# ejcanalesr/multicomponent-T2-toolbox

Hardware: AMD Instinct MI355X
Metric: voxels/sec (whole node) at nTE=32, nT2=60; max |MWF-ref| (higher is better)
Workload: dtype f64

## Files before the change

### include/met2_hip.h

```cpp
#ifndef MET2_HIP_H
#define MET2_HIP_H

#include <stdint.h>

#ifdef __cplusplus
extern "C" {
#endif

#define MET2_ABI_VERSION 6

enum met2_method {
    MET2_NNLS = 0,
    MET2_T2SPARC = 1,
    MET2_X2 = 2,
    MET2_LCURVE = 3,
    MET2_GCV = 4,
    MET2_BAYESREG = 5
};

enum met2_penalty { MET2_PEN_I = 0, MET2_PEN_L1 = 1, MET2_PEN_L2 = 2, MET2_PEN_INVT2 = 3 };

enum met2_status {
    MET2_ST_FITTED = 1,
    MET2_ST_ITMAX = 2,
// ... 112 lines not shown
int met2_fa_bruteforce_strided(met2_plan *plan, int64_t nvox, const double *data, int64_t voxel_stride, int64_t echo_stride,
                               const uint8_t *mask, double *fa_index, double *km, double *resid, void *stream);

int met2_fa_spline_select(int32_t device, int64_t nvox, int32_t n_lr, const double *alpha_lr, const double *resid,
                          int32_t n_hr, const double *alpha_hr, int32_t n_te, const double *data, const uint8_t *mask,
                          double *fa_index, double *xmin, void *stream);

int met2_fa_spline_select_strided(int32_t device, int64_t nvox, int32_t n_lr, const double *alpha_lr, const double *resid,
                                  int32_t n_hr, const double *alpha_hr, int32_t n_te, const double *data, int64_t voxel_stride,
                                  int64_t echo_stride, const uint8_t *mask, double *fa_index, double *xmin, void *stream);

int met2_smooth_separable(int32_t device, int32_t nx, int32_t ny, int32_t nz, int32_t n_te, int32_t radius, const double *weights,
                          const double *data, double *out, double *work, void *stream);

int met2_nesma(int32_t device, int32_t nx, int32_t ny, int32_t nz, int32_t n_te, const double *data,
               const uint8_t *mask, double *out, void *stream);

int64_t met2_tv_work_bytes(int32_t nx, int32_t ny, int32_t nz, int32_t n_te, int32_t echo_major);
int met2_tv_chambolle(int32_t device, int32_t nx, int32_t ny, int32_t nz, int32_t n_te, const double *data, int32_t echo_major,
                      const double *weight, double weight_factor, double eps, int32_t max_num_iter, int32_t poll_every, double *out,
                      double *sigma, int32_t *iters, void *work, int64_t work_bytes, void *stream);
int met2_tv_last_timing(double *iter_ms, int32_t *launches);

int met2_roi_reduce(met2_plan *src, met2_plan *dst, int64_t nvox, const double *data, int64_t voxel_stride, int64_t echo_stride,
                    const int32_t *roi_index, const double *fa_index, double *mean_signal, double *count, void *stream);

int met2_metrics(met2_plan *plan, int64_t nvox, const double *fsol, const uint8_t *mask, double *maps,
                 void *stream);

int met2_plan_last_kernel_ms(met2_plan *plan, double *ms);
int met2_plan_last_spill_count(met2_plan *plan, int64_t *count);
int met2_plan_last_second_pass_ms(met2_plan *plan, double *ms);

int met2_plan_launch_info(met2_plan *plan, int32_t method, int32_t *grid, int32_t *block, int32_t *lds_bytes);

int met2_plan_gcv_form(met2_plan *plan, int32_t *low_rank, double *residual);

#ifdef __cplusplus
}
#endif
#endif
```

### multicomponent-t2-toolbox_amd/_lib.py

```python
import ctypes as C
import os

from . import _build

_LIB = None

_dp = C.POINTER(C.c_double)


class Met2Error(RuntimeError):
    pass


class Options(C.Structure):
    _fields_ = [("struct_size", C.c_int32), ("device", C.c_int32), ("x2_factor", C.c_double), ("t2sparc_lambda", C.c_double),
                ("brent_xtol", C.c_double), ("brent_maxfun", C.c_int32), ("reserved0", C.c_int32), ("t2_myelin_cut", C.c_double),
                ("t2_ie_cut", C.c_double), ("x2_lo", C.c_double), ("x2_hi", C.c_double), ("gcv_lo", C.c_double), ("gcv_hi", C.c_double),
                ("bayes_lo", C.c_double), ("bayes_hi", C.c_double)]


class SynthParams(C.Structure):
    _fields_ = [("struct_size", C.c_int32), ("reserved0", C.c_int32), ("te", C.c_double), ("TR", C.c_double), ("T1", C.c_double)] + [
        (k, C.c_double) for k in ("mwf_lo", "mwf_hi", "t2m_lo", "t2m_hi", "t2ie_lo", "t2ie_hi", "fa_lo", "fa_hi", "snr_lo", "snr_hi", "sm_lo", "sm_hi",
                                  "sie_lo", "sie_hi", "km")]


SYMBOLS = ["met2_default_options", "met2_abi_version", "met2_device_count", "met2_last_error", "met2_plan_create",
           "met2_plan_destroy", "met2_plan_set_options", "met2_plan_get_options", "met2_plan_build_dictionary_epg", "met2_plan_set_dictionary", "met2_plan_get_dictionary",
           "met2_plan_set_penalty", "met2_plan_set_penalty_dense", "met2_plan_get_penalty", "met2_plan_set_lambda_grid",
           "met2_plan_set_t2_grid", "met2_fit", "met2_fit_strided", "met2_fit_enqueue_strided", "met2_plan_finish", "met2_fa_bruteforce", "met2_fa_bruteforce_strided", "met2_fa_spline_select",
           "met2_fa_spline_select_strided", "met2_roi_reduce", "met2_nesma", "met2_tv_work_bytes", "met2_tv_chambolle", "met2_tv_last_timing", "met2_smooth_separable", "met2_metrics", "met2_plan_last_kernel_ms", "met2_plan_last_second_pass_ms", "met2_plan_last_spill_count",
           "met2_plan_launch_info", "met2_plan_gcv_form", "met2_plan_get_shape", "met2_fit_host", "met2_plan_attach_fa_spline", "met2_host_trim",
           "met2_fit_bootstrap", "met2_bootstrap_replicates", "met2_synth_two_lobe", "met2_eval_voxel_metrics", "met2_eval_reduce"]


def lib():
    global _LIB
    if _LIB is None:
        path = _build.LIB
        if not os.path.exists(path):
            raise Met2Error("HIP extension %s is not built (run __graft_entry__.build()); there is no CPU fallback" % path)
        L = C.CDLL(path)
        L.met2_last_error.restype = C.c_char_p
        vp = C.c_void_p
        L.met2_plan_create.argtypes = [C.POINTER(vp), C.c_int32, C.c_int32, C.c_int32, C.POINTER(Options)]
        L.met2_plan_destroy.argtypes = [vp]
        L.met2_plan_set_options.argtypes = [vp, C.POINTER(Options)]
        L.met2_plan_get_options.argtypes = [vp, C.POINTER(Options)]
        L.met2_plan_build_dictionary_epg.argtypes = [vp, _dp, _dp, C.c_double, _dp, C.c_double, vp]
        L.met2_plan_set_dictionary.argtypes = [vp, _dp]
        L.met2_plan_get_dictionary.argtypes = [vp, _dp]
        L.met2_plan_set_penalty.argtypes = [vp, C.c_int32, _dp]
        L.met2_plan_set_penalty_dense.argtypes = [vp, _dp]
        L.met2_plan_get_penalty.argtypes = [vp, _dp]
        L.met2_plan_set_lambda_grid.argtypes = [vp, _dp, C.c_int32]
        L.met2_plan_set_t2_grid.argtypes = [vp, _dp]
        L.met2_fit.argtypes = [vp, C.c_int32, C.c_int64] + [vp] * 10
        L.met2_fit_strided.argtypes = [vp, C.c_int32, C.c_int64, vp, C.c_int64, C.c_int64] + [vp] * 9
        L.met2_fit_enqueue_strided.argtypes = [vp, C.c_int32, C.c_int64, vp, C.c_int64, C.c_int64] + [vp] * 9
        L.met2_plan_finish.argtypes = [vp, vp]
        L.met2_fa_bruteforce.argtypes = [vp, C.c_int64] + [vp] * 6
        L.met2_fa_bruteforce_strided.argtypes = [vp, C.c_int64, vp, C.c_int64, C.c_int64] + [vp] * 5
        L.met2_fa_spline_select_strided.argtypes = [C.c_int32, C.c_int64, C.c_int32, _dp, vp, C.c_int32, _dp, C.c_int32, vp, C.c_int64, C.c_int64,
                                                    vp, vp, vp, vp]
        L.met2_roi_reduce.argtypes = [vp, vp, C.c_int64, vp, C.c_int64, C.c_int64, vp, vp, vp, vp, vp]
        L.met2_fa_spline_select.argtypes = [C.c_int32, C.c_int64, C.c_int32, _dp, vp, C.c_int32, _dp, C.c_int32, vp, vp, vp, vp, vp]
        L.met2_nesma.argtypes = [C.c_int32] * 5 + [vp] * 4
        L.met2_tv_work_bytes.argtypes = [C.c_int32] * 5
        L.met2_tv_work_bytes.restype = C.c_int64
        L.met2_tv_chambolle.argtypes = [C.c_int32] * 5 + [vp, C.c_int32, _dp, C.c_double, C.c_double, C.c_int32, C.c_int32, vp, vp, vp, vp, C.c_int64, vp]
        L.met2_tv_last_timing.argtypes = [_dp, C.POINTER(C.c_int32)]
        L.met2_smooth_separable.argtypes = [C.c_int32] * 6 + [_dp] + [vp] * 4
        L.met2_metrics.argtypes = [vp, C.c_int64, vp, vp, vp, vp]
        L.met2_plan_last_kernel_ms.argtypes = [vp, _dp]
        L.met2_plan_last_second_pass_ms.argtypes = [vp, _dp]
        L.met2_plan_last_spill_count.argtypes = [vp, C.POINTER(C.c_int64)]
        L.met2_plan_gcv_form.argtypes = [vp, C.POINTER(C.c_int32), _dp]
        L.met2_plan_launch_info.argtypes = [vp, C.c_int32, C.POINTER(C.c_int32), C.POINTER(C.c_int32), C.POINTER(C.c_int32)]
        L.met2_plan_get_shape.argtypes = [vp, C.POINTER(C.c_int32), C.POINTER(C.c_int32), C.POINTER(C.c_int32)]
        L.met2_fit_host.argtypes = [C.POINTER(vp), C.c_int32, C.c_int32, C.c_int64, vp, vp, C.c_int64, C.c_int64, vp, vp, vp, C.c_int32] + [vp] * 8 + [C.c_int64, _dp]
        L.met2_host_trim.argtypes = []
        L.met2_plan_attach_fa_spline.argtypes = [vp, vp, C.c_int32, _dp, C.c_int32, _dp]
        L.met2_fit_bootstrap.argtypes = [vp, C.c_int32, C.c_int64, vp, C.c_int64, C.c_int64, vp, vp, vp, vp, C.c_int32, C.c_int64] + [vp] * 10
        L.met2_bootstrap_replicates.argtypes = [vp, C.c_int64, vp, vp, vp, C.c_int32, C.c_int64, vp, vp]
        L.met2_synth_two_lobe.argtypes = [vp, C.POINTER(SynthParams), C.c_int64, C.c_int64, C.c_int64, vp, vp, vp, vp]
        L.met2_eval_voxel_metrics.argtypes = [vp, C.c_int64, vp, vp, vp, vp]
        L.met2_eval_reduce.argtypes = [C.c_int64, vp, vp, vp, vp, vp, vp]
        _LIB = L
    return _LIB


def check(rc):
    if rc != 0:
        msg = lib().met2_last_error()
        raise Met2Error("met2_hip error %d: %s" % (rc, msg.decode() if msg else "?"))
```

### multicomponent-t2-toolbox_amd/csrc/fit_kernel.hpp

```cpp
#pragma once
#include <hip/hip_runtime.h>
#include <math.h>
#include <stdint.h>

#include "../../include/met2_hip.h"
#include "abi_common.hpp"
#include "nnls_wave.hpp"
#include "objectives.hpp"

using namespace met2;

struct SortBufs {
    int *key;
    int *perm;
    int *hist;
    int *cursor;
    int *bucket_start;
    int *chunk_start;
    int *queue;
    int *xq;
    int *err;
    int *ovf;
};

// ... 8 lines not shown
    int wave_doubles;
    int method, nlam, maxfun;
    double x2_factor, t2sparc_lambda, xtol;
    double cut_m, cut_ie;
    double lam_lo, lam_hi;
    int all_queued;
    double log_detL;
    const double *Dfa;
    const double *Bfa;
    const double *Dtfa;
    const double *Aq;
    const double *kband;
    const double *lband;
    const double *Kd;
    const double *lam_grid;
    const double *t2s;
    const double *data;
    int64_t vs, es;
    SortBufs sb;
    double *fsol, *sig, *reg, *lam, *maps;
    int32_t *status;
    int64_t nvox;
    const char *seed;
    const double *btab;
    int nbtab, btab_stride;
    double *chol;
    int chol_stride;
    double *big;
    int big_stride;
    double *lc_save;
    int *lc_at;
    int lc_cap;
    double blam[MET2_BAYES_TABLE];
};

#ifndef MET2_UNI_MASK
#define MET2_UNI_MASK 37
#endif
constexpr bool uni_brent(int method, int nb)
{
    const int base = method >= 10 ? method - 10 : method;
    const int bit = base == MET2_X2 ? 0 : ((base == MET2_GCV || base == MET2_GCV_LR) ? 2 : (base == MET2_BAYESREG ? 4 : -1));
    return bit >= 0 && ((MET2_UNI_MASK >> (bit + (nb == 2 ? 1 : 0))) & 1);
}
template <bool PIN>
__device__ __forceinline__ double uni(double v)
{
    if constexpr (PIN) {
    const unsigned long long u = (unsigned long long)__double_as_longlong(v);
    const unsigned lo = (unsigned)__builtin_amdgcn_readfirstlane((int)(unsigned)u), hi = (unsigned)__builtin_amdgcn_readfirstlane((int)(unsigned)(u >> 32));
    return __longlong_as_double((long long)(((unsigned long long)hi << 32) | lo));
    } else return v;
}
#define MET2_UNI_PIN() do { a = uni<PIN>(a); b = uni<PIN>(b); fulc = uni<PIN>(fulc); nfc = uni<PIN>(nfc); xf = uni<PIN>(xf); rat = uni<PIN>(rat); e = uni<PIN>(e); \
                            x = uni<PIN>(x); fx = uni<PIN>(fx); ffulc = uni<PIN>(ffulc); fnfc = uni<PIN>(fnfc); } while (0)

template <bool PIN, class F, class G>
__device__ __forceinline__ double fminbound_dev(F &&fn, G &&on_best, double x1, double x2, double xatol, int maxfun, int &flag)
{
    const double sqrt_eps = sqrt(2.2e-16);
    const double golden_mean = 0.5 * (3.0 - sqrt(5.0));
    double a = x1, b = x2;
    double fulc = a + golden_mean * (b - a);
    double nfc = fulc, xf = fulc;
    double rat = 0.0, e = 0.0;
    double x = xf;
// ... 646 lines not shown
        if (NB == 2 && lane + 64 < n) A.fsol[(size_t)v * n + lane + 64] = 0.0;
        if (lane == 0) { A.reg[v] = 0.0; if (A.status) A.status[v] = stat | (overflow ? MET2_ST_KOVERFLOW : 0); }
        return false;
    }
    if (st.itmax_hit & 1) stat |= MET2_ST_ITMAX;
    if (st.itmax_hit & 2) stat |= MET2_ST_KOVERFLOW;
    MET2_CYC_END(0, c_vox);
    MET2_CYC_FLUSH(st);

    double xs[NB];
#pragma unroll
    for (int bb = 0; bb < NB; ++bb) {
        xs[bb] = st.x[bb] * km;
        if (lane + 64 * bb < n) A.fsol[(size_t)v * n + lane + 64 * bb] = xs[bb]; else xs[bb] = 0.0;
    }
    if (A.sig) {
        double sg = model_signal<NB>(S, st, lane) * km;
        if (lane < m) A.sig[(size_t)v * m + lane] = sg;
    }
    if (A.maps) write_metrics<NB>(ml, xs, true, A.maps, A.nvox, v, lane);
    if (lane == 0) {
        A.reg[v] = regv;
        if (A.lam) A.lam[v] = lamv;
        if (A.status) A.status[v] = stat;
    }
    return !BIG && !queued && (st.itmax_hit & 2) != 0;
}

__device__ __forceinline__ void fit_shared(const FitArgs &A, WaveShared &S, double *sR, int wslot)
{
    S.R = sR; S.n = A.n; S.m = A.m; S.kmax = A.kmax; S.rcap = A.wave_doubles; S.K = A.Kd; S.kband = A.kband; S.Dt = nullptr; S.DtG = A.Dtfa; S.dtstride = A.m; S.buffer_rows = true; S.reorder = true; S.have_bdiag = false; S.bdiag[0] = S.bdiag[1] = 0.0;
    S.B = A.Bfa; S.D = A.Dfa; S.bstride = A.n; S.dstride = A.n;
    S.Rg = A.big ? A.big + (size_t)wslot * (size_t)A.big_stride : nullptr; S.gbase = col_base(A.kmax);
}
template <int METHOD>
__device__ __forceinline__ void fit_shared_fa(const FitArgs &A, WaveShared &S, int fa)
{
    const int n = A.n, m = A.m;
    S.B = A.Bfa + (size_t)fa * n * n; S.D = A.Dfa + (size_t)fa * m * n; S.Dt = A.Dtfa + (size_t)fa * m * n;
    S.DtG = ((METHOD >= 10 ? METHOD - 10 : METHOD) == MET2_GCV_LR) ? A.Aq + (size_t)fa * n * MET2_GCV_LR_RANK : S.Dt;
}

template <int METHOD, int NB>
__device__ __attribute__((noinline)) void fit_voxel_spill(const FitArgs *Ap, big_lds_dp sRl, int64_t v, int fa, int wslot, int qslot, int seed_cap)
{
    const int lane = big_lane();
    double *sR = (double *)sRl;
    FitArgs A;
    {
        static_assert(sizeof(FitArgs) % 4 == 0, "FitArgs is copied word by word");
        const int *src = (const int *)Ap;
        int *dst = (int *)&A;
#pragma unroll
        for (int i = 0; i < (int)(sizeof(FitArgs) / 4); ++i) dst[i] = big_rfl(src[i]);
    }
    v = (int64_t)big_rfl((u64)v); fa = big_rfl(fa); wslot = big_rfl(wslot); qslot = big_rfl(qslot); seed_cap = big_rfl(seed_cap);
    WaveShared S;
    fit_shared(A, S, sR, wslot);
    fit_shared_fa<METHOD>(A, S, fa);
    Band<NB> bd;
    load_band<NB>(bd, A.kband, A.lband, lane);
    MetricLanes<NB> ml;
    metric_lanes<NB>(ml, A.t2s, A.n, A.cut_m, A.cut_ie, lane);
    const int seed_k = (MET2_SEED && A.seed) ? ((const SeedRec *)A.seed)[fa].k : 0;
    const bool have_seed = seed_k > 0 && seed_k <= seed_cap;
    (void)fit_voxel<METHOD, NB, true>(A, S, bd, ml, v, fa, seed_k, have_seed, lane, wslot, qslot);
// ... 94 lines not shown
```

### multicomponent-t2-toolbox_amd/csrc/met2_fit_nnls_lcurve.hip

```cpp
#ifdef MET2_SPLIT_TU
#include "fit_kernel.hpp"
template int launch_fit_nb<0, 1, false>(const FitArgs &, const LaunchGeom &, hipStream_t);
template int launch_fit_nb<0, 2, false>(const FitArgs &, const LaunchGeom &, hipStream_t);
template int launch_fit_nb<1, 1, false>(const FitArgs &, const LaunchGeom &, hipStream_t);
template int launch_fit_nb<1, 2, false>(const FitArgs &, const LaunchGeom &, hipStream_t);
template int launch_fit_nb<3, 1, false>(const FitArgs &, const LaunchGeom &, hipStream_t);
template int launch_fit_nb<3, 2, false>(const FitArgs &, const LaunchGeom &, hipStream_t);
template int launch_fit_nb<0, 1, true>(const FitArgs &, const LaunchGeom &, hipStream_t);
template int launch_fit_nb<0, 2, true>(const FitArgs &, const LaunchGeom &, hipStream_t);
template int launch_fit_nb<1, 1, true>(const FitArgs &, const LaunchGeom &, hipStream_t);
template int launch_fit_nb<1, 2, true>(const FitArgs &, const LaunchGeom &, hipStream_t);
template int launch_fit_nb<3, 1, true>(const FitArgs &, const LaunchGeom &, hipStream_t);
template int launch_fit_nb<3, 2, true>(const FitArgs &, const LaunchGeom &, hipStream_t);
#endif
```

### multicomponent-t2-toolbox_amd/csrc/met2_fit_x2_nb1.hip

```cpp
#ifdef MET2_SPLIT_TU
#include "fit_kernel.hpp"
template int launch_fit_nb<2, 1, false>(const FitArgs &, const LaunchGeom &, hipStream_t);
template int launch_fit_nb<12, 1, false>(const FitArgs &, const LaunchGeom &, hipStream_t);
#endif
```

### multicomponent-t2-toolbox_amd/csrc/met2_hip.hip

```cpp
#include <hip/hip_runtime.h>
#include <math.h>
#include <stddef.h>
#include <stdint.h>
#include <stdio.h>
#include <stdlib.h>
#include <string.h>
#include <string>
#include <vector>

#include "../../include/met2_hip.h"
#include "abi_common.hpp"
#include "nnls_wave.hpp"
#include "objectives.hpp"
#include "fit_kernel.hpp"

using namespace met2;

#ifdef MET2_SPLIT_TU
extern template int launch_fit_nb<0, 1, false>(const FitArgs &, const LaunchGeom &, hipStream_t);
extern template int launch_fit_nb<0, 2, false>(const FitArgs &, const LaunchGeom &, hipStream_t);
extern template int launch_fit_nb<1, 1, false>(const FitArgs &, const LaunchGeom &, hipStream_t);
extern template int launch_fit_nb<1, 2, false>(const FitArgs &, const LaunchGeom &, hipStream_t);
extern template int launch_fit_nb<2, 1, false>(const FitArgs &, const LaunchGeom &, hipStream_t);
extern template int launch_fit_nb<2, 2, false>(const FitArgs &, const LaunchGeom &, hipStream_t);
// ... 787 lines not shown

__global__ __launch_bounds__(256) void roi_finish_kernel(RoiArgs A)
{
    extern __shared__ int roi_tot[];
    __shared__ double s_nv;
    const int r = (int)blockIdx.x;
    for (int f = threadIdx.x; f < A.nfa; f += blockDim.x) {
        int c = 0;
        for (int sl = 0; sl < A.nslice; ++sl) c += A.part_cnt[((size_t)r * A.nslice + sl) * A.nfa + f];
        roi_tot[f] = c;
    }
    __syncthreads();
    if (threadIdx.x == 0) {
        long long nv = 0;
        for (int f = 0; f < A.nfa; ++f) nv += roi_tot[f];
        s_nv = (double)nv;
        A.count[r] = (double)nv;
    }
    __syncthreads();
    const double nv = s_nv;
    if ((int)threadIdx.x < A.nte) {
        double t = 0.0;
        for (int sl = 0; sl < A.nslice; ++sl) t += A.part_sig[((size_t)r * A.nslice + sl) * 64 + threadIdx.x];
        A.mean_sig[(size_t)r * A.nte + threadIdx.x] = t / nv;
    }
    const int sz = A.nte * A.nt2;
    for (int i = threadIdx.x; i < sz; i += blockDim.x) {
        double t = 0.0;
        for (int f = 0; f < A.nfa; ++f) { const int c = roi_tot[f]; if (c) t = fma((double)c, A.Dsrc[(size_t)f * sz + i], t); }
        A.Ddst[(size_t)r * sz + i] = t / nv;
    }
}

struct met2_plan {
    int n_te, n_t2, n_fa;
    met2_options opt;
    int cus;
    double *dD = nullptr;
    double *dB = nullptr;
    double *dKband = nullptr;
    double *dLband = nullptr;
    double *dDt = nullptr;
    double *dKd = nullptr;
    double *dLam = nullptr;
    double *dT2 = nullptr;
    int nlam = 0;
    bool have_dict = false, have_pen = false, have_t2 = false;
    std::vector<double> Lhost;
    double log_detL = 0.0;
    int64_t cap_vox = 0;
    int *dKey = nullptr, *dPerm = nullptr, *dSmall = nullptr, *dOvf = nullptr;
    char *dSeed = nullptr;
    bool seeds_valid = false; double seeds_key[7] = {0};
    bool seeds_ok = false;
    double *dH = nullptr; int64_t cap_h = 0;
    double *dBtab = nullptr; int btab_stride = 0;
    double *dQt = nullptr;
    double *dAq = nullptr, *dAqRes = nullptr;
    double gcv_res = 0.0;
    bool gcv_lr = false;
    double *dChol = nullptr; int64_t cap_chol = 0;
    double *dLcSave = nullptr; int64_t cap_lc = 0;
    double *dBig = nullptr; int64_t cap_big = 0;
    int last_spill = 0;
    double blam[MET2_BAYES_TABLE > 0 ? MET2_BAYES_TABLE : 1];
    int *hErr = nullptr;
// ... 822 lines not shown
        if (sort_lds > 150 * 1024) return fail(MET2_E_UNSUPPORTED, "more than 19 000 flip angles (or ROIs) in one plan");
        HIPCHK(hipFuncSetAttribute((const void *)classify_kernel, hipFuncAttributeMaxDynamicSharedMemorySize, (int)sort_lds));
        HIPCHK(hipFuncSetAttribute((const void *)scatter_kernel, hipFuncAttributeMaxDynamicSharedMemorySize, (int)sort_lds));
        HIPCHK(hipFuncSetAttribute((const void *)scan_kernel, hipFuncAttributeMaxDynamicSharedMemorySize, (int)sort_lds));
    }
    int chunk = (method <= MET2_T2SPARC) ? 8 : 1;
    chunk = tuning_env("MET2_CHUNK", 1, 1024, chunk);
    const bool dbg = test_switch("MET2_DEBUG");
    if (dbg) { HIPCHK(hipStreamSynchronize(s)); fprintf(stderr, "[met2] fit: nvox=%lld grid=%d block=%d lds=%d\n", (long long)nvox, g.grid, g.block, g.lds); fflush(stderr); }
    hipLaunchKernelGGL(classify_kernel, dim3(nbs), dim3(MET2_SORT_BLOCK), sort_lds, s, nvox, p->n_te, p->n_fa, data, voxel_stride, echo_stride, fa_index, mask, 1, sb, status);
    hipLaunchKernelGGL(scan_kernel, dim3(1), dim3(256), sort_lds, s, p->n_fa, chunk, sb);
    if (dbg) { HIPCHK(hipStreamSynchronize(s)); fprintf(stderr, "[met2] classify done\n"); fflush(stderr); }
    hipLaunchKernelGGL(scatter_kernel, dim3(nbs), dim3(MET2_SORT_BLOCK), sort_lds, s, nvox, p->n_fa, sb);
    HIPCHK(hipGetLastError());
    if (dbg) {
        HIPCHK(hipStreamSynchronize(s));
        std::vector<int> hs(4 * (size_t)(p->n_fa + 1) + 8);
        HIPCHK(hipMemcpy(hs.data(), p->dSmall, sizeof(int) * hs.size(), hipMemcpyDeviceToHost));
        fprintf(stderr, "[met2] sort done: fitted=%d chunks=%d\n", hs[2 * (p->n_fa + 1) + p->n_fa], hs[3 * (p->n_fa + 1) + p->n_fa]); fflush(stderr);
    }

    FitArgs A;
    A.n = p->n_t2; A.m = p->n_te; A.nfa = p->n_fa; A.kmax = g.kmax; A.waves = g.waves; A.chunk = chunk; A.wave_doubles = g.wave_doubles;
    A.method = method; A.nlam = p->nlam;
    A.maxfun = p->opt.brent_maxfun > 0 ? p->opt.brent_maxfun : (method == MET2_BAYESREG ? 200 : 300);
    A.x2_factor = p->opt.x2_factor; A.t2sparc_lambda = p->opt.t2sparc_lambda; A.xtol = p->opt.brent_xtol;
    A.cut_m = p->opt.t2_myelin_cut; A.cut_ie = p->opt.t2_ie_cut;
    A.lam_lo = method == MET2_GCV ? p->opt.gcv_lo : (method == MET2_BAYESREG ? p->opt.bayes_lo : p->opt.x2_lo);
    A.lam_hi = method == MET2_GCV ? p->opt.gcv_hi : (method == MET2_BAYESREG ? p->opt.bayes_hi : p->opt.x2_hi);
    A.log_detL = p->log_detL;
    A.Dfa = p->dD; A.Bfa = p->dB; A.Dtfa = p->dDt; A.Aq = p->dAq; A.kband = p->dKband; A.lband = p->dLband; A.Kd = p->dKd; A.lam_grid = p->dLam; A.t2s = p->dT2;
    A.data = data; A.vs = voxel_stride; A.es = echo_stride; A.sb = sb; A.fsol = fsol; A.sig = sig; A.reg = reg; A.lam = lam; A.maps = maps; A.status = status; A.nvox = nvox;

    A.seed = nullptr;
    if (!test_switch("MET2_NO_SEED") && !objgrid && p->have_pen && p->seeds_valid && p->seeds_ok && p->seeds_key[0] == p->opt.t2sparc_lambda &&
        (method == MET2_X2 || method == MET2_GCV || method == MET2_BAYESREG || method == MET2_T2SPARC)) {
        const int slot = method == MET2_BAYESREG ? 1 : (method == MET2_T2SPARC ? 2 : (method == MET2_GCV ? 3 : 0));
        A.seed = p->dSeed + sizeof(SeedRec) * (size_t)slot * p->n_fa;
    }
    A.btab = nullptr; A.nbtab = 0; A.btab_stride = p->btab_stride;
    A.chol = nullptr; A.chol_stride = 0;
    if (method == MET2_BAYESREG && !objgrid && g.nb == 2) {
        const int stride = (col_base(p->n_t2) + 15) & ~15;
        const int64_t need = (int64_t)g.grid * g.waves * stride;
        if (p->cap_chol < need) {
            if (p->dChol) { HIPCHK(hipStreamSynchronize(s)); HIPCHK(hipFree(p->dChol)); p->dChol = nullptr; p->cap_chol = 0; }
            HIPCHK(hipMalloc(&p->dChol, sizeof(double) * (size_t)need));
            p->cap_chol = need;
        }
        A.chol = p->dChol; A.chol_stride = stride;
    }
    A.big = nullptr; A.big_stride = 0;
    if (kfast) {
        const int stride = (col_base(p->n_t2) - col_base(g.kmax) + 15) & ~15;
        LaunchGeom gw;
        rc = fit_geometry(p, kmeth, gw, kfast, 0, -1);
        if (rc) return rc;
        const int64_t need = (int64_t)gw.grid * gw.waves * stride;
        if (p->cap_big < need) {
            if (p->dBig) { HIPCHK(hipStreamSynchronize(s)); HIPCHK(hipFree(p->dBig)); p->dBig = nullptr; p->cap_big = 0; }
            HIPCHK(hipMalloc(&p->dBig, sizeof(double) * (size_t)need));
            p->cap_big = need;
        }
        A.big = p->dBig; A.big_stride = stride;
    }
    A.lc_save = nullptr; A.lc_at = nullptr; A.lc_cap = 0;
// ... 207 lines not shown
    *ms = (double)f;
    return MET2_OK;
}

int met2_plan_last_spill_count(met2_plan *p, int64_t *count)
{
    if (!p || !count) return fail(MET2_E_INVALID, "NULL argument");
    *count = p->last_spill;
    return MET2_OK;
}

int met2_plan_last_second_pass_ms(met2_plan *p, double *ms)
{
    if (!p || !ms) return fail(MET2_E_INVALID, "NULL argument");
    *ms = 0.0;
    if (!p->timed || !p->timed2) return MET2_OK;
    USE_DEVICE(p->opt.device);
    HIPCHK(hipEventSynchronize(p->ev2));
    float f = 0.f;
    HIPCHK(hipEventElapsedTime(&f, p->ev1, p->ev2));
    *ms = (double)f;
    return MET2_OK;
}

int met2_plan_gcv_form(met2_plan *p, int32_t *low_rank, double *residual)
{
    if (!p) return fail(MET2_E_INVALID, "NULL plan");
    if (!p->have_dict) return fail(MET2_E_STATE, "no dictionary in the plan");
    if (low_rank) *low_rank = kernel_method(p, MET2_GCV) == MET2_GCV_LR ? 1 : 0;
    if (residual) *residual = p->gcv_res;
    return MET2_OK;
}

int met2_plan_launch_info(met2_plan *p, int32_t method, int32_t *grid, int32_t *block, int32_t *lds_bytes)
{
    if (!p) return fail(MET2_E_INVALID, "NULL plan");
    LaunchGeom g;
    method = kernel_method(p, method);
    const int kf = fast_kmax(p, method);
    int rc = fit_geometry(p, method, g, kf);
    if (rc) return rc;
    if (grid) *grid = g.grid;
    if (block) *block = g.block;
    if (lds_bytes) *lds_bytes = g.lds;
    return MET2_OK;
}

}
```

### multicomponent-t2-toolbox_amd/csrc/nnls_wave.hpp

```cpp
#pragma once
#include "wave_ops.hpp"

namespace met2 {

#ifndef MET2_DOUBLE
#define MET2_DOUBLE 0
#endif
#ifndef MET2_REORDER
#define MET2_REORDER 2
#endif

#ifdef MET2_LOOPSTATS
__device__ int g_loopstats[8];
#define MET2_STAT(slot, v) atomicMax(&g_loopstats[slot], (int)(v))
#else
#define MET2_STAT(slot, v)
#endif

#ifdef MET2_CYCSTATS
__device__ unsigned long long g_cyc[16];
__device__ unsigned long long g_ev[40][12];
#define MET2_CYC_BEGIN(var) const unsigned long long var = __builtin_readcyclecounter()
#define MET2_CYC_END(slot, var) st.cyc[slot] += __builtin_readcyclecounter() - var
#define MET2_CYC_ADD(slot, v) st.cyc[slot] += (unsigned long long)(v)
#define MET2_CYC_INIT(st) do { for (int q_ = 0; q_ < 16; ++q_) st.cyc[q_] = 0; } while (0)
#define MET2_CYC_FLUSH(st) do { if (lane_id() == 0) for (int q_ = 0; q_ < 16; ++q_) atomicAdd(&g_cyc[q_], st.cyc[q_]); } while (0)
#else
#define MET2_CYC_BEGIN(var)
#define MET2_CYC_END(slot, var)
#define MET2_CYC_ADD(slot, v)
#define MET2_CYC_INIT(st)
#define MET2_CYC_FLUSH(st)
#endif

struct WaveShared {
    const double *B;
    const double *K;
    const double *Dt;
    const double *DtG;
    const double *kband;
    int dtstride;
    const double *D;
    double *R;
    int n, m, bstride, dstride, kmax;
    int rcap;
    bool have_bdiag;
    double bdiag[2];
    bool reorder;
    bool buffer_rows;
    double *Rg = nullptr;
    int gbase = 0;
};

template <int NB>
struct Band {
    double lb[NB][5];
};

template <int NB>
struct NnlsState {
    double h[NB];
    double x[NB];
    int pos[NB];
    double y[NB];
    double rinv[NB];
    int ord[NB];
    int k;
    u64 P[NB];
    int itmax_hit;
#ifdef MET2_CYCSTATS
    unsigned long long cyc[16];
#endif
};

__device__ __forceinline__ int row_base(int i, int kmax) { return i * kmax - (i * (i - 1)) / 2 - i; }
__host__ __device__ __forceinline__ constexpr int col_len(int c) { return c + 1; }
__host__ __device__ __forceinline__ constexpr int col_base(int c) { return (c * (c + 1)) >> 1; }

typedef double met2_d2 __attribute__((ext_vector_type(2)));
typedef double met2_d4 __attribute__((ext_vector_type(4)));
typedef const volatile __attribute__((address_space(3))) double *met2_lds_cvp;
__device__ __forceinline__ void lds_quad(const double *p, double &a, double &b, double &c, double &d)
{
    met2_lds_cvp q = (met2_lds_cvp)p;
// ... 87 lines not shown
__device__ __forceinline__ void shifted(const double (&v)[NB], int d, int lane, double (&below)[NB], double (&above)[NB])
{
    const int lm = (lane - d) & 63, lp = (lane + d) & 63;
    double lo_m = gather(v[0], lm), lo_p = gather(v[0], lp);
    if (NB == 1) { below[0] = lo_m; above[0] = lo_p; return; }
    double hi_m = gather(v[NB - 1], lm), hi_p = gather(v[NB - 1], lp);
    below[0] = lo_m;
    below[NB - 1] = (lane >= d) ? hi_m : lo_m;
    above[0] = (lane + d < 64) ? lo_p : hi_p;
    above[NB - 1] = hi_p;
}

template <int NB>
__device__ __forceinline__ void band_mul(const double (&bnd)[NB][5], const double (&v)[NB], int lane, double (&out)[NB])
{
    double m1[NB], p1[NB], m2[NB], p2[NB];
    shifted<NB>(v, 1, lane, m1, p1);
    shifted<NB>(v, 2, lane, m2, p2);
#pragma unroll
    for (int b = 0; b < NB; ++b)
        out[b] = bnd[b][2] * v[b] + bnd[b][0] * m2[b] + bnd[b][1] * m1[b] + bnd[b][3] * p1[b] + bnd[b][4] * p2[b];
}

__device__ __forceinline__ double ld_row(const double *array_base, int row_off_elems, unsigned lane_off_bytes)
{
    const __amdgpu_buffer_rsrc_t r = __builtin_amdgcn_make_buffer_rsrc((void *)array_base, 0, 0x40000000, 0x00020000);
    const auto v = __builtin_amdgcn_raw_buffer_load_b64(r, lane_off_bytes, (unsigned)row_off_elems * 8u, 0);
    return __hiloint2double((int)v[1], (int)v[0]);
}

__device__ __forceinline__ double ld_row_sel(bool buffer, const double *array_base, int row_off_elems, unsigned lane_elem)
{
    return buffer ? ld_row(array_base, row_off_elems, 8u * lane_elem) : array_base[row_off_elems + (int)lane_elem];
}

__device__ __forceinline__ double rsqrt_nr(double d)
{
    const double r = __builtin_amdgcn_rsq(d);
    const double e = fma(-(0.5 * d) * r, r, 0.5);
    return fma(r, e * fma(1.5, e, 1.0), r);
}

__device__ __forceinline__ double rcp_nr(double d)
{
    const double r = __builtin_amdgcn_rcp(d);
    const double e = fma(-d, r, 1.0);
    return fma(r, fma(e, e, e), r);
}

__device__ __forceinline__ void givens(double a, double b, double &c, double &s, double &sig, double &rinv)
{
    const double r2 = fma(a, a, b * b);
    if (r2 > 0.0) { rinv = rsqrt_nr(r2); c = a * rinv; s = b * rinv; sig = r2 * rinv; }
    else { sig = 0.0; c = 0.0; s = 1.0; rinv = INFINITY; }
}

template <int NB, int NP = NB>
__device__ __forceinline__ void back_subst(const WaveShared &S, const NnlsState<NB> &st, int lane, double (&z)[NB])
{
    const int k = st.k;
    double y[NB], ra[NB], rb[NB];
    int cb = col_base(k - 1);
#pragma unroll
    for (int b = 0; b < NP; ++b) {
        const int pl = lane + 64 * b;
        y[b] = st.y[b];
// ... 441 lines not shown
        MET2_STAT(2, outer + 1);
        MET2_STAT(3, iter);
    }
    return true;
}

#ifndef MET2_ONE_SLOT
#define MET2_ONE_SLOT 1
#endif
template <int NB, int ONE = 0, bool BIG = false>
__device__ __forceinline__ void nnls_iterate(const WaveShared &S, const Band<NB> &bd, NnlsState<NB> &st, double lam, int mrows, int lane,
                                             bool warm = false)
{
    if constexpr (NB == 2 && ONE == 1 && MET2_ONE_SLOT) {
        int iter = 0, outer = 0;
        if (st.k <= 63 && iterate_leg<NB, 1, BIG>(S, bd, st, lam, mrows, lane, warm, iter, outer)) return;
        if constexpr (BIG) {
            if (st.k <= S.kmax && iterate_leg<NB, NB, true>(S, bd, st, lam, mrows, lane, warm, iter, outer)) return;
            if (S.Rg) iterate_big<NB>(S, bd, st, lam, mrows, lane, warm, iter, outer);
        } else
            (void)iterate_leg<NB, NB>(S, bd, st, lam, mrows, lane, warm, iter, outer);
    } else
        nnls_iterate_plain<NB, (NB == 2 && ONE == 3), BIG>(S, bd, st, lam, mrows, lane, warm);
}

template <int NB>
__device__ __forceinline__ void nnls_reset(NnlsState<NB> &st)
{
#pragma unroll
    for (int b = 0; b < NB; ++b) { st.x[b] = 0.0; st.y[b] = 0.0; st.rinv[b] = 0.0; st.ord[b] = 0; st.pos[b] = -1; st.P[b] = 0ull; }
    st.k = 0;
}

template <int NB, int NP = NB>
__device__ __forceinline__ bool refactor_rowwise(const WaveShared &S, const Band<NB> &bd, NnlsState<NB> &st, double lam, int lane)
{
    const int k = st.k, n = S.n;
    int cbl[NB], cbc[NB];
    unsigned jc[NB];
    double g[NB], gb0[NB], gk0[NB], gb1[NB], gk1[NB];
#pragma unroll
    for (int b = 0; b < NB; ++b) {
        const int pl = lane + 64 * b;
        jc[b] = (unsigned)min(pl, n - 1);
        if (b < NP) {
            cbl[b] = col_base(pl);
            cbc[b] = col_base(min(pl, k - 1));
            const double hh = gatherN<NB>(st.h, st.ord[b]);
            g[b] = (pl < k) ? hh : 0.0;
        }
    }
    auto fetch = [&](int p, double (&vb)[NB], double (&vk)[NB]) {
        const int t = bcastPos_i<NB, NP>(st.ord, min(p, k - 1));
#pragma unroll
        for (int b = 0; b < NB; ++b) {
            vb[b] = ld_row_sel(S.buffer_rows, S.B, t * S.bstride, jc[b]);
            vk[b] = ld_row_sel(S.buffer_rows, S.K, t * n, jc[b]);
        }
    };
    auto finish = [&](int i, double (&a)[NB], double (&r)[NB]) {
        const double d = bcastPos<NB, NP>(a, i);
        const double rinv = rsqrt_nr(d);
        const double yi = bcastPos<NB, NP>(g, i) * rinv;
#pragma unroll
        for (int b = 0; b < NP; ++b) {
            const int pl = lane + 64 * b;
            r[b] = a[b] * rinv;
            if (pl >= i && pl < k) S.R[cbl[b] + i] = r[b];
            g[b] = (pl > i) ? fma(-r[b], yi, g[b]) : g[b];
        }
    };
    double gdp[NB];
    {
        double gdb[NB];
#pragma unroll
        for (int b = 0; b < NB; ++b) {
            const double bd0 = S.have_bdiag ? S.bdiag[b] : S.B[jc[b] * S.bstride + jc[b]];
            gdb[b] = (lam != 0.0) ? fma(lam, S.K[jc[b] * n + jc[b]], bd0) : bd0;
        }
#pragma unroll
        for (int b = 0; b < NP; ++b) gdp[b] = gatherN<NB>(gdb, st.ord[b]);
    }
    fetch(0, gb0, gk0);
    fetch(1, gb1, gk1);
    int cbi = 0;
    bool bad = false;
    int i = 0;
    for (; i + 1 < k; i += 2) {
        double a[NB], c[NB];
        {
            double t0[NB], t1[NB];
#pragma unroll
            for (int b = 0; b < NB; ++b) { t0[b] = fma(lam, gk0[b], gb0[b]); t1[b] = fma(lam, gk1[b], gb1[b]); }
            fetch(i + 2, gb0, gk0);
            fetch(i + 3, gb1, gk1);
#pragma unroll
            for (int b = 0; b < NP; ++b) { a[b] = gatherN<NB>(t0, st.ord[b]); c[b] = gatherN<NB>(t1, st.ord[b]); }
        }
        const double *ci = S.R + cbi, *cj = ci + col_len(i);
        int j = 0;
#pragma clang loop unroll(disable)
        for (; j + 4 <= i; j += 4) {
            double s0, s1, s2, s3, u0, u1, u2, u3;
            lds_quad(ci + j, s0, s1, s2, s3);
            lds_quad(cj + j, u0, u1, u2, u3);
#pragma unroll
            for (int b = 0; b < NP; ++b) {
                double q0, q1, q2, q3;
                lds_quad(S.R + cbc[b] + j, q0, q1, q2, q3);
                a[b] = fma(-s0, q0, a[b]); c[b] = fma(-u0, q0, c[b]);
                a[b] = fma(-s1, q1, a[b]); c[b] = fma(-u1, q1, c[b]);
                a[b] = fma(-s2, q2, a[b]); c[b] = fma(-u2, q2, c[b]);
                a[b] = fma(-s3, q3, a[b]); c[b] = fma(-u3, q3, c[b]);
            }
        }
        if (j + 2 <= i) {
            double s0, s1, u0, u1;
            lds_pair(ci + j, s0, s1);
            lds_pair(cj + j, u0, u1);
#pragma unroll
// ... 239 lines not shown
#pragma unroll
                for (int sidx = 0; sidx < 4; ++sidx) acc = __builtin_amdgcn_mfma_f64_16x16x4f64(aop[sidx], bop[sidx], acc, 0, 0, 0);
#pragma unroll
                for (int v = 0; v < 4; ++v) {
                    const int row = 16 * ti + lk + 4 * v;
                    if (cc < k && row <= cc) S.R[cbb + row] = acc[v];
                }
            }
        }
        __builtin_amdgcn_wave_barrier();
    }
    bool bad = false;
    double dgl[NB];
#pragma unroll
    for (int b = 0; b < NB; ++b) {
        const int pl = lane + 64 * b;
        dgl[b] = (pl < k) ? S.R[cbl[b] + pl] : 1.0;
        bad = bad || (ballot((pl < k) && !(dgl[b] * dgl[b] > 1e-14 * gdp[b])) != 0ull);
    }
    if (bad) return false;
#pragma unroll
    for (int b = 0; b < NB; ++b) {
        const int pl = lane + 64 * b;
        const double ri = rcp_nr(dgl[b]);
        st.rinv[b] = (pl < k) ? ri : st.rinv[b];
        st.y[b] = (pl < k) ? g[b] * ri : st.y[b];
    }
    return true;
}

#ifndef MET2_ONE_SLOT_REFACTOR
#define MET2_ONE_SLOT_REFACTOR 1
#endif
#ifndef MET2_REFACTOR_BLOCKED_FROM
#define MET2_REFACTOR_BLOCKED_FROM 2
#endif
template <int NB, int ONE = 0, bool BIG = false>
__device__ __forceinline__ bool refactor(const WaveShared &S, const Band<NB> &bd, NnlsState<NB> &st, double lam, int lane)
{
    if constexpr (BIG) if (st.k > S.kmax) return refactor_big<NB>(S, bd, st, lam, lane);
    if (NB == 2 && ONE && MET2_ONE_SLOT && MET2_ONE_SLOT_REFACTOR && st.k <= 64) return refactor_rowwise<NB, 1>(S, bd, st, lam, lane);
    if (NB >= MET2_REFACTOR_BLOCKED_FROM) return refactor_blocked<NB>(S, bd, st, lam, lane);
    if (MET2_DOUBLE == 1) { (void)refactor_rowwise<NB>(S, bd, st, lam, lane); __builtin_amdgcn_wave_barrier(); }
    return refactor_rowwise<NB>(S, bd, st, lam, lane);
}

template <int NB, int ONE = 0, bool BIG = false>
__device__ __forceinline__ void nnls_solve(const WaveShared &S, const Band<NB> &bd, NnlsState<NB> &st, double lam, bool aug, int lane)
{
    nnls_reset<NB>(st);
    nnls_iterate<NB, ONE, BIG>(S, bd, st, lam, aug ? S.m + S.n : S.m, lane);
}

template <int NB>
__device__ __forceinline__ void reorder_by_x(const WaveShared &S, NnlsState<NB> &st, int lane)
{
    const int k = st.k;
    typedef __attribute__((address_space(3))) unsigned long long *lds_u64p;
    unsigned long long *tabk = (unsigned long long *)S.R;
    int *tabi = (int *)(tabk + k + 4);
    unsigned long long key[NB];
    bool in[NB];
#pragma unroll
    for (int b = 0; b < NB; ++b) {
        const int j = lane + 64 * b;
        in[b] = (st.P[b] >> lane) & 1ull;
        key[b] = ((unsigned long long)__double_as_longlong(st.x[b]) & ~127ull) | (unsigned long long)(127 - j);
        if (in[b]) tabk[st.pos[b]] = key[b];
        if (j >= k && j < k + 4) tabk[j] = 0ull;
    }
    __builtin_amdgcn_wave_barrier();
    int rank[NB];
#pragma unroll
    for (int b = 0; b < NB; ++b) rank[b] = 0;
#pragma clang loop unroll(disable)
    for (int p = 0; p < k; p += 4) {
        const unsigned long long k0 = tabk[p], k1 = tabk[p + 1], k2 = tabk[p + 2], k3 = tabk[p + 3];
// ... 276 lines not shown
```

Baseline: 6.862 million.

## Pack two column pairs per wave in NB=1 rowwise Cholesky refactor

Adds a packed path to the rowwise refactorization for one-bin-per-lane waves when the active set size is between 4 and 32. The upper and lower 32 lanes each process a separate column pair, so four columns advance per iteration instead of two. The goal is to use the otherwise idle half of the wave and halve the number of serial outer iterations. The cost is extra cross-lane broadcasts, extra barriers and more complex indexing, with a risk of numerical or correctness mistakes in the hand-written second-half update. It also adds an optional debug counter and a pair-mode switch, both controlled by environment variables.

Result: faster. 7.223 million, median of 6 (+5.3%).

```diff
diff --git a/include/met2_hip.h b/include/met2_hip.h
--- a/include/met2_hip.h
+++ b/include/met2_hip.h
@@ -168,6 +168,8 @@
 int met2_plan_last_spill_count(met2_plan *plan, int64_t *count);
 int met2_plan_last_second_pass_ms(met2_plan *plan, double *ms);
 
+int met2_refac_packed_calls(met2_plan *plan, uint64_t *calls, int32_t reset);
+
 int met2_plan_launch_info(met2_plan *plan, int32_t method, int32_t *grid, int32_t *block, int32_t *lds_bytes);
 
 int met2_plan_gcv_form(met2_plan *plan, int32_t *low_rank, double *residual);
diff --git a/multicomponent-t2-toolbox_amd/_lib.py b/multicomponent-t2-toolbox_amd/_lib.py
--- a/multicomponent-t2-toolbox_amd/_lib.py
+++ b/multicomponent-t2-toolbox_amd/_lib.py
@@ -31,7 +31,7 @@
            "met2_plan_set_t2_grid", "met2_fit", "met2_fit_strided", "met2_fit_enqueue_strided", "met2_plan_finish", "met2_fa_bruteforce", "met2_fa_bruteforce_strided", "met2_fa_spline_select",
            "met2_fa_spline_select_strided", "met2_roi_reduce", "met2_nesma", "met2_tv_work_bytes", "met2_tv_chambolle", "met2_tv_last_timing", "met2_smooth_separable", "met2_metrics", "met2_plan_last_kernel_ms", "met2_plan_last_second_pass_ms", "met2_plan_last_spill_count",
            "met2_plan_launch_info", "met2_plan_gcv_form", "met2_plan_get_shape", "met2_fit_host", "met2_plan_attach_fa_spline", "met2_host_trim",
-           "met2_fit_bootstrap", "met2_bootstrap_replicates", "met2_synth_two_lobe", "met2_eval_voxel_metrics", "met2_eval_reduce"]
+           "met2_fit_bootstrap", "met2_bootstrap_replicates", "met2_synth_two_lobe", "met2_eval_voxel_metrics", "met2_eval_reduce", "met2_refac_packed_calls"]
 
 
 def lib():
@@ -76,6 +76,7 @@
         L.met2_plan_last_second_pass_ms.argtypes = [vp, _dp]
         L.met2_plan_last_spill_count.argtypes = [vp, C.POINTER(C.c_int64)]
         L.met2_plan_gcv_form.argtypes = [vp, C.POINTER(C.c_int32), _dp]
+        L.met2_refac_packed_calls.argtypes = [vp, C.POINTER(C.c_uint64), C.c_int32]
         L.met2_plan_launch_info.argtypes = [vp, C.c_int32, C.POINTER(C.c_int32), C.POINTER(C.c_int32), C.POINTER(C.c_int32)]
         L.met2_plan_get_shape.argtypes = [vp, C.POINTER(C.c_int32), C.POINTER(C.c_int32), C.POINTER(C.c_int32)]
         L.met2_fit_host.argtypes = [C.POINTER(vp), C.c_int32, C.c_int32, C.c_int64, vp, vp, C.c_int64, C.c_int64, vp, vp, vp, C.c_int32] + [vp] * 8 + [C.c_int64, _dp]
diff --git a/multicomponent-t2-toolbox_amd/csrc/fit_kernel.hpp b/multicomponent-t2-toolbox_amd/csrc/fit_kernel.hpp
--- a/multicomponent-t2-toolbox_amd/csrc/fit_kernel.hpp
+++ b/multicomponent-t2-toolbox_amd/csrc/fit_kernel.hpp
@@ -64,6 +64,8 @@
     int *lc_at;
     int lc_cap;
     double blam[MET2_BAYES_TABLE];
+    int refac_pair = 0;
+    unsigned long long *refac_count = nullptr;
 };
 
 #ifndef MET2_UNI_MASK
@@ -776,6 +778,7 @@
     S.R = sR; S.n = A.n; S.m = A.m; S.kmax = A.kmax; S.rcap = A.wave_doubles; S.K = A.Kd; S.kband = A.kband; S.Dt = nullptr; S.DtG = A.Dtfa; S.dtstride = A.m; S.buffer_rows = true; S.reorder = true; S.have_bdiag = false; S.bdiag[0] = S.bdiag[1] = 0.0;
     S.B = A.Bfa; S.D = A.Dfa; S.bstride = A.n; S.dstride = A.n;
     S.Rg = A.big ? A.big + (size_t)wslot * (size_t)A.big_stride : nullptr; S.gbase = col_base(A.kmax);
+    S.refac_pair = A.refac_pair != 0; S.refac_count = A.refac_count;
 }
 template <int METHOD>
 __device__ __forceinline__ void fit_shared_fa(const FitArgs &A, WaveShared &S, int fa)
diff --git a/multicomponent-t2-toolbox_amd/csrc/met2_fit_nnls_lcurve.hip b/multicomponent-t2-toolbox_amd/csrc/met2_fit_nnls_lcurve.hip
--- a/multicomponent-t2-toolbox_amd/csrc/met2_fit_nnls_lcurve.hip
+++ b/multicomponent-t2-toolbox_amd/csrc/met2_fit_nnls_lcurve.hip
@@ -1,4 +1,5 @@
 #ifdef MET2_SPLIT_TU
+#define MET2_REFAC_PACKED 1
 #include "fit_kernel.hpp"
 template int launch_fit_nb<0, 1, false>(const FitArgs &, const LaunchGeom &, hipStream_t);
 template int launch_fit_nb<0, 2, false>(const FitArgs &, const LaunchGeom &, hipStream_t);
diff --git a/multicomponent-t2-toolbox_amd/csrc/met2_fit_x2_nb1.hip b/multicomponent-t2-toolbox_amd/csrc/met2_fit_x2_nb1.hip
--- a/multicomponent-t2-toolbox_amd/csrc/met2_fit_x2_nb1.hip
+++ b/multicomponent-t2-toolbox_amd/csrc/met2_fit_x2_nb1.hip
@@ -1,4 +1,5 @@
 #ifdef MET2_SPLIT_TU
+#define MET2_REFAC_PACKED 1
 #include "fit_kernel.hpp"
 template int launch_fit_nb<2, 1, false>(const FitArgs &, const LaunchGeom &, hipStream_t);
 template int launch_fit_nb<12, 1, false>(const FitArgs &, const LaunchGeom &, hipStream_t);
diff --git a/multicomponent-t2-toolbox_amd/csrc/met2_hip.hip b/multicomponent-t2-toolbox_amd/csrc/met2_hip.hip
--- a/multicomponent-t2-toolbox_amd/csrc/met2_hip.hip
+++ b/multicomponent-t2-toolbox_amd/csrc/met2_hip.hip
@@ -843,6 +843,8 @@
     }
 }
 
+__device__ unsigned long long g_refac_packed_calls;
+
 struct met2_plan {
     int n_te, n_t2, n_fa;
     met2_options opt;
@@ -1731,6 +1733,9 @@
     A.Dfa = p->dD; A.Bfa = p->dB; A.Dtfa = p->dDt; A.Aq = p->dAq; A.kband = p->dKband; A.lband = p->dLband; A.Kd = p->dKd; A.lam_grid = p->dLam; A.t2s = p->dT2;
     A.data = data; A.vs = voxel_stride; A.es = echo_stride; A.sb = sb; A.fsol = fsol; A.sig = sig; A.reg = reg; A.lam = lam; A.maps = maps; A.status = status; A.nvox = nvox;
 
+    A.refac_pair = test_switch("MET2_REFAC_PAIR") ? 1 : 0;
+    A.refac_count = nullptr;
+    if (test_switch("MET2_REFAC_COUNT")) HIPCHK(hipGetSymbolAddress((void **)&A.refac_count, HIP_SYMBOL(g_refac_packed_calls)));
     A.seed = nullptr;
     if (!test_switch("MET2_NO_SEED") && !objgrid && p->have_pen && p->seeds_valid && p->seeds_ok && p->seeds_key[0] == p->opt.t2sparc_lambda &&
         (method == MET2_X2 || method == MET2_GCV || method == MET2_BAYESREG || method == MET2_T2SPARC)) {
@@ -2004,6 +2009,18 @@
     return MET2_OK;
 }
 
+int met2_refac_packed_calls(met2_plan *p, uint64_t *calls, int32_t reset)
+{
+    if (!p) return fail(MET2_E_INVALID, "NULL plan");
+    USE_DEVICE(p->opt.device);
+    HIPCHK(hipDeviceSynchronize());
+    unsigned long long v = 0;
+    HIPCHK(hipMemcpyFromSymbol(&v, HIP_SYMBOL(g_refac_packed_calls), sizeof(v)));
+    if (calls) *calls = (uint64_t)v;
+    if (reset) { v = 0; HIPCHK(hipMemcpyToSymbol(HIP_SYMBOL(g_refac_packed_calls), &v, sizeof(v))); }
+    return MET2_OK;
+}
+
 int met2_plan_launch_info(met2_plan *p, int32_t method, int32_t *grid, int32_t *block, int32_t *lds_bytes)
 {
     if (!p) return fail(MET2_E_INVALID, "NULL plan");
diff --git a/multicomponent-t2-toolbox_amd/csrc/nnls_wave.hpp b/multicomponent-t2-toolbox_amd/csrc/nnls_wave.hpp
--- a/multicomponent-t2-toolbox_amd/csrc/nnls_wave.hpp
+++ b/multicomponent-t2-toolbox_amd/csrc/nnls_wave.hpp
@@ -50,6 +50,8 @@
     bool buffer_rows;
     double *Rg = nullptr;
     int gbase = 0;
+    bool refac_pair = false;
+    unsigned long long *refac_count = nullptr;
 };
 
 template <int NB>
@@ -203,6 +205,11 @@
 __device__ __forceinline__ double ld_row_sel(bool buffer, const double *array_base, int row_off_elems, unsigned lane_elem)
 {
     return buffer ? ld_row(array_base, row_off_elems, 8u * lane_elem) : array_base[row_off_elems + (int)lane_elem];
+}
+
+__device__ __forceinline__ double ld_elem_sel(bool buffer, const double *array_base, unsigned elem)
+{
+    return buffer ? ld_row(array_base, 0, 8u * elem) : array_base[elem];
 }
 
 __device__ __forceinline__ double rsqrt_nr(double d)
@@ -710,9 +717,10 @@
     st.k = 0;
 }
 
-template <int NB, int NP = NB>
+template <int NB, int NP = NB, bool PACK = false>
 __device__ __forceinline__ bool refactor_rowwise(const WaveShared &S, const Band<NB> &bd, NnlsState<NB> &st, double lam, int lane)
 {
+    static_assert(!PACK || (NB == 1 && NP == 1), "the packed leg is written for one bin per lane");
     const int k = st.k, n = S.n;
     int cbl[NB], cbc[NB];
     unsigned jc[NB];
@@ -759,11 +767,88 @@
 #pragma unroll
         for (int b = 0; b < NP; ++b) gdp[b] = gatherN<NB>(gdb, st.ord[b]);
     }
-    fetch(0, gb0, gk0);
-    fetch(1, gb1, gk1);
     int cbi = 0;
     bool bad = false;
     int i = 0;
+    bool packed = false;
+    if constexpr (PACK) {
+    packed = k >= 4 && k <= 32 && !S.refac_pair;
+    if (packed) {
+        if (S.refac_count && lane == 0) atomicAdd(S.refac_count, 1ull);
+        const int lo_ = lane_opaque(lane), hi2 = (lo_ >> 5) << 1, cp = lo_ & 31;
+        const int cbq = col_base(min(cp, k - 1));
+        auto fetch_packed = [&](int p0) {
+            const unsigned oc = (unsigned)gather_i(st.ord[0], min(lane_opaque(lane) & 31, k - 1));
+            const unsigned ta = (unsigned)gather_i(st.ord[0], min(p0 + hi2, k - 1)), tb = (unsigned)gather_i(st.ord[0], min(p0 + hi2 + 1, k - 1));
+            gb0[0] = ld_elem_sel(S.buffer_rows, S.B, ta * (unsigned)S.bstride + oc);
+            gk0[0] = ld_elem_sel(S.buffer_rows, S.K, ta * (unsigned)n + oc);
+            gb1[0] = ld_elem_sel(S.buffer_rows, S.B, tb * (unsigned)S.bstride + oc);
+            gk1[0] = ld_elem_sel(S.buffer_rows, S.K, tb * (unsigned)n + oc);
+        };
+        fetch_packed(0);
+        for (; i + 3 < k; i += 4) {
+            double a[NB], c[NB];
+            a[0] = fma(lam, gk0[0], gb0[0]); c[0] = fma(lam, gk1[0], gb1[0]);
+            const int ih = i + hi2;
+            const double *ci = S.R + col_base(ih), *cj = ci + col_len(ih), *cq = S.R + cbq;
+#pragma clang loop unroll(disable)
+            for (int j = 0; j < i; j += 2) {
+                double s0, s1, u0, u1, q0, q1;
+                lds_pair(ci + j, s0, s1);
+                lds_pair(cj + j, u0, u1);
+                lds_pair(cq + j, q0, q1);
+                a[0] = fma(-s0, q0, a[0]); c[0] = fma(-u0, q0, c[0]);
+                a[0] = fma(-s1, q1, a[0]); c[0] = fma(-u1, q1, c[0]);
+            }
+            if (i + 7 < k) fetch_packed(i + 4);
+            else { fetch(i + 4, gb0, gk0); fetch(i + 5, gb1, gk1); }
+            {
+                double r[NB], r1[NB];
+                finish(i, a, r);
+                const double sr = bcast(r[0], i + 1);
+                double cl[NB];
+                cl[0] = fma(-sr, r[0], c[0]);
+                finish(i + 1, cl, r1);
+            }
+            __builtin_amdgcn_wave_barrier();
+            {
+                double s0, s1, u0, u1, q0, q1;
+                lds_pair(ci + i, s0, s1);
+                lds_pair(cj + i, u0, u1);
+                lds_pair(cq + i, q0, q1);
+                a[0] = fma(-s0, q0, a[0]); c[0] = fma(-u0, q0, c[0]);
+                a[0] = fma(-s1, q1, a[0]); c[0] = fma(-u1, q1, c[0]);
+            }
+            const int iu = i + 2;
+            double y2, y3;
+            {
+                const double rinv2 = rsqrt_nr(bcast(a[0], 32 + iu));
+                y2 = bcast(g[0], iu) * rinv2;
+                const double r2 = a[0] * rinv2;
+                if (lane >= 32 + iu && lane < 32 + k) S.R[cbq + iu] = r2;
+                const double sr = bcast(r2, 32 + iu + 1);
+                c[0] = fma(-sr, r2, c[0]);
+                const double rinv3 = rsqrt_nr(bcast(c[0], 32 + iu + 1));
+                y3 = fma(-sr, y2, bcast(g[0], iu + 1)) * rinv3;
+                const double r3 = c[0] * rinv3;
+                if (lane >= 32 + iu + 1 && lane < 32 + k) S.R[cbq + iu + 1] = r3;
+            }
+            __builtin_amdgcn_wave_barrier();
+            {
+                double e2, e3;
+                lds_pair(cq + iu, e2, e3);
+                g[0] = (lane > iu) ? fma(-e2, y2, g[0]) : g[0];
+                g[0] = (lane > iu + 1) ? fma(-e3, y3, g[0]) : g[0];
+            }
+            __builtin_amdgcn_wave_barrier();
+        }
+        cbi = col_base(i);
+    }
+    }
+    if (!packed) {
+        fetch(0, gb0, gk0);
+        fetch(1, gb1, gk1);
+    }
     for (; i + 1 < k; i += 2) {
         double a[NB], c[NB];
         {
@@ -1069,6 +1154,12 @@
 #ifndef MET2_ONE_SLOT_REFACTOR
 #define MET2_ONE_SLOT_REFACTOR 1
 #endif
+#if !defined(MET2_REFAC_PACKED) && !defined(MET2_SPLIT_TU)
+#define MET2_REFAC_PACKED 1
+#endif
+#ifndef MET2_REFAC_PACKED
+#define MET2_REFAC_PACKED 0
+#endif
 #ifndef MET2_REFACTOR_BLOCKED_FROM
 #define MET2_REFACTOR_BLOCKED_FROM 2
 #endif
@@ -1078,8 +1169,9 @@
     if constexpr (BIG) if (st.k > S.kmax) return refactor_big<NB>(S, bd, st, lam, lane);
     if (NB == 2 && ONE && MET2_ONE_SLOT && MET2_ONE_SLOT_REFACTOR && st.k <= 64) return refactor_rowwise<NB, 1>(S, bd, st, lam, lane);
     if (NB >= MET2_REFACTOR_BLOCKED_FROM) return refactor_blocked<NB>(S, bd, st, lam, lane);
-    if (MET2_DOUBLE == 1) { (void)refactor_rowwise<NB>(S, bd, st, lam, lane); __builtin_amdgcn_wave_barrier(); }
-    return refactor_rowwise<NB>(S, bd, st, lam, lane);
+    constexpr bool PACK = MET2_REFAC_PACKED && NB == 1 && !BIG;
+    if (MET2_DOUBLE == 1) { (void)refactor_rowwise<NB, NB, PACK>(S, bd, st, lam, lane); __builtin_amdgcn_wave_barrier(); }
+    return refactor_rowwise<NB, NB, PACK>(S, bd, st, lam, lane);
 }
 
 template <int NB, int ONE = 0, bool BIG = false>
```
